# openai/Video-Pre-Training

Hardware: AMD Instinct MI355X
Metric: frames/sec (fwd) [+ bc_step.ms_per_step], 2x policy, 128x128x3 seq=128 (higher is better)
Workload: dtype bf16; 1 GPU; foundation-model-2x policy forward (IMPALA CNN + 4-layer banded transformer + heads), batch=64 seq=128 uint8 128x128x3 frames per GPU, KV memory carried, random-init weights; global_batch=64, seq_len=128, parallelism=dp1 replicas (no collective in forward; BC step: gradient all-reduce)

## Files before the change

video-pre-training_amd/csrc/vpt_conv3x3_fwd.hip:

```cpp
#include "vpt_conv3x3_tile.h"
#include <type_traits>
#ifndef VPT_EPI_NO_CLAMP_RELU
#define VPT_EPI_NO_CLAMP_RELU 0
#endif
#if defined(VPT_CONV_PROFILE) && defined(VPT_CONV_FWD_ABLATE)
#define FWD_NO_DMA (VPT_CONV_FWD_ABLATE == 1 || VPT_CONV_FWD_ABLATE == 4)
#define FWD_NO_HALO (VPT_CONV_FWD_ABLATE == 2 || VPT_CONV_FWD_ABLATE == 4)
#else
#define FWD_NO_DMA 0
#define FWD_NO_HALO 0
#endif
template <int U> __device__ __forceinline__ f32x4 ac_get(const f32x16& v) {
  return __builtin_shufflevector(v, v, 4 * U, 4 * U + 1, 4 * U + 2, 4 * U + 3);
}
template <int U> __device__ __forceinline__ void ac_set(f32x16& v, const f32x4 c) {
  const f32x16 w = __builtin_shufflevector(c, c, 0, 1, 2, 3, -1, -1, -1, -1, -1, -1, -1, -1, -1, -1, -1, -1);
  if constexpr (U == 0) v = __builtin_shufflevector(v, w, 16, 17, 18, 19, 4, 5, 6, 7, 8, 9, 10, 11, 12, 13, 14, 15);
  else if constexpr (U == 1) v = __builtin_shufflevector(v, w, 0, 1, 2, 3, 16, 17, 18, 19, 8, 9, 10, 11, 12, 13, 14, 15);
  else if constexpr (U == 2) v = __builtin_shufflevector(v, w, 0, 1, 2, 3, 4, 5, 6, 7, 16, 17, 18, 19, 12, 13, 14, 15);
  else v = __builtin_shufflevector(v, w, 0, 1, 2, 3, 4, 5, 6, 7, 8, 9, 10, 11, 16, 17, 18, 19);
}

template <bool TRACE, int MODE, int TR = 16, bool HDMA = false>
__global__ __launch_bounds__(TR * 16, 2) void vpt_conv3x3_kernel(VptConv3x3Args a) {
// ... 29 lines not shown
  const int tilesX = a.W >> 4, tilesY = a.H / TR;
  const VptConvTile tile = conv_tile_decode(a.NT, tilesX, tilesY);
  const int nt = tile.nt, tx = tile.tx, ty = tile.ty, f = tile.f;
  const int tx0 = tx * 16, ty0 = ty * TR;
  const int NCB = a.Cin >> 5;
  const int HW = a.H * a.W;

  int a_loff[NA];
  unsigned a_gbyte[NA];
  unsigned a_inside = 0;
#pragma unroll
  for (int m = 0; m < NA; ++m) {
    const int q = tid + NTHR * m;
    const int P = ((q >> 5) << 3) + 2 * (q & 3) + ((q >> 4) & 1);
    const int part = 2 * ((q >> 3) & 1) + ((q >> 2) & 1);
    a_loff[m] = -1;
    a_gbyte[m] = 0u;
    if (P < HPIX) {
      const int hy = P / 18, hx = P - hy * 18;
      const int y = ty0 - 1 + hy, x = tx0 - 1 + hx;
      a_loff[m] = P * A_RS + part * 16 + 16 * (P & 1);
      if (y >= 0 && y < a.H && x >= 0 && x < a.W) {
        a_gbyte[m] = (unsigned)((y * a.W + x) * 32 + part * 8) * 2u;
        a_inside |= 1u << m;
      }
    }
  }
  const op16_t* xplane = a.x + (size_t)f * NCB * HW * 32;
  constexpr int H16_STR = (NTHR / 4) * A_RS;
  static_assert(((NA - 2) * NTHR + NTHR - 1) / 32 * 8 + 7 < HPIX, "all chunks but a thread's last are inside the halo");
  const int a_l0 = a_loff[0];
  const bool a_lastok = a_loff[NA - 1] >= 0;
  const op16_t* wbase = a.wpk + (size_t)nt * NCB * 9 * 4096 + (size_t)(w * 64 + lane) * 8;
  unsigned char* bdst = smem + A_SZ + w * 1024;
  unsigned hv[6] = {0u, 0u, 0u, 0u, 0u, 0u};
  if constexpr (HDMA) {
#pragma unroll
    for (int n = 0; n < 6; ++n) {
      const int s = (n < 5 ? (4 * n + w) * 64 : (H_BUF - 1024) / 16) + lane;
      const int P = s >> 2, hy = P / 18, hx = P - 18 * hy;
      const int q = (s & 3) ^ ((hx >> 2) & 3);
      const int y = ty0 - 1 + hy, x = tx0 - 1 + hx;
      hv[n] = (y >= 0 && y < a.H && x >= 0 && x < a.W) ? (unsigned)((y * a.W + x) * 64 + q * 16) : H_OOB;
    }
  }
  const unsigned h_wbytes = (unsigned)NCB * 9u * (unsigned)H_SLOT, h_xbytes = (unsigned)NCB * (unsigned)HW * 64u;
  const op16_t* const h_wptr = a.wpk + (size_t)nt * NCB * 9 * 4096;
  const __amdgpu_buffer_rsrc_t hwrs = __builtin_amdgcn_make_buffer_rsrc((void*)h_wptr, 0, HDMA ? h_wbytes : 0u, 0x00020000);
  const __amdgpu_buffer_rsrc_t hxrs = __builtin_amdgcn_make_buffer_rsrc((void*)xplane, 0, HDMA ? h_xbytes : 0u, 0x00020000);
  const int h_wvoff = (w * 64 + lane) * 16;
  unsigned char* const rdst = smem + w * 1024;
  int h_wso = 0, h_rpi = 0;

#define GLDS16(m_)                                                                                        \
  do { if (POOL) { if (!FWD_NO_DMA) GLDS(m_); } else if ((m_) < NDMA && !FWD_NO_DMA)                      \
  __builtin_amdgcn_raw_ptr_buffer_load_lds(wrs, (__attribute__((address_space(3))) void*)(bd_ + (m_) * (NWAVE * 1024)), 16, wvoff, \
                                           (s_ + 1) * B_BYTES + (m_) * (NWAVE * 1024), 0, 0); } while (0)
#define XA16(m_) do { if (!FWD_NO_HALO) XA(m_); } while (0)
#define HALO_WR16(m_) do { if ((m_) < NA - 1 || a_lastok) *(u32x4*)(smem + a_l0 + (m_) * H16_STR) = ((a_inside >> (m_)) & 1u) ? areg[m_] : zero4; } while (0)
#define PA(j_, dy_, dx_) fp[j_] = *(const __attribute__((address_space(3))) op16x8*)((((dx_) & 1) ? aLo : aLe) + (((j_) + (dy_)) * 18 + (dx_)) * A_RS)
#define WB(tap_, u_, boff_) fw[(u_) & 1] = *(const __attribute__((address_space(3))) op16x8*)((((u_) & 1) ? bW1 : bW0) + (boff_) + (tap_) * (128 * 64) + ((u_) >> 1) * (32 * 64))
#define M16A(j_, u_) ac_set<(u_)>(ac[j_], VPT_MFMA_16X16X32(fw[(u_) & 1], fp[j_], ac_get<(u_)>(ac[j_]), 0, 0, 0))
#define G16(MM_, u_, WLD, X)                                                                              \
  do {                                                                                                    \
    MM_(0, u_); WLD; SB();                                                                                \
    MM_(1, u_); SB();                                                                                     \
    MM_(2, u_); SB();                                                                                     \
    MM_(3, u_); X; SB();                                                                                  \
    MM_(4, u_); SB();                                                                                     \
    MM_(5, u_); SB();                                                                                     \
    MM_(6, u_); SB();                                                                                     \
    MM_(7, u_); SB();                                                                                     \
  } while (0)
#define G16R(MM_, WLD, X, ndy_, ndx_)                                                                     \
  do {                                                                                                    \
    MM_(0, 3); SB(); WLD; PA(0, ndy_, ndx_); SB();                                                              \
    MM_(1, 3); SB(); PA(1, ndy_, ndx_); SB();                                                                   \
    MM_(2, 3); SB(); PA(2, ndy_, ndx_); SB();                                                                   \
    MM_(3, 3); SB(); PA(3, ndy_, ndx_); X; SB();                                                                \
    MM_(4, 3); SB(); PA(4, ndy_, ndx_); SB();                                                                   \
    MM_(5, 3); SB(); PA(5, ndy_, ndx_); SB();                                                                   \
    MM_(6, 3); SB(); PA(6, ndy_, ndx_); SB();                                                                   \
    MM_(7, 3); SB(); PA(7, ndy_, ndx_); SB();                                                                   \
  } while (0)
#define TAP16(MM_, dy_, dx_, X0, X1, X2, X3)                                                              \
  do {                                                                                                    \
    G16(MM_, 0, WB(dx_, 1, boff_), X0);                                                                   \
    G16(MM_, 1, WB(dx_, 2, boff_), X1);                                                                   \
    G16(MM_, 2, WB(dx_, 3, boff_), X2);                                                                   \
    G16R(MM_, WB((dx_) + 1, 0, boff_), X3, dy_, (dx_) + 1);                                               \
  } while (0)
#define EPI_LD16(ptr_, j_, n2_) (*(const u32x4*)((const char*)((ptr_) + cbase[n2_]) + (voff16 + (unsigned)(j_) * gj_b)))
#define XR16(j_) do { rq16[j_][0] = EPI_LD16(resp, j_, 0); rq16[j_][1] = EPI_LD16(resp, j_, 1); } while (0)
#define XR16L(j_) do { rq16[j_][0] = *(const u32x4*)((const char*)(resp + cbase[0]) + (voff16_l + (unsigned)(j_) * gj_b)); rq16[j_][1] = *(const u32x4*)((const char*)(resp + cbase[1]) + (voff16_l + (unsigned)(j_) * gj_b)); } while (0)
#define CONV_STEP16(cb_, dy_, NEXT_DY, PRE_A, WR_A, PRE_R, LAST)                                          \
  do {                                                                                                    \
    const int s_ = (cb_) * 3 + (dy_);                                                                     \
    const int boff_ = (s_ & 1) * B_BYTES, noff_ = B_BYTES - boff_;                                        \
    const op16_t* wp_ = wbase + (size_t)(s_ + 1) * 12288;      \
    unsigned char* bd_ = bdst + noff_;                                                                    \
    const unsigned cbo_ = (unsigned)((cb_) + 1) * (unsigned)HW * 64u;                 \
    if (LAST) {                                                                                           \
      TAP16(M16A, dy_, 0, NOP_(), NOP_(), NOP_(), NOP_());                                                \
    } else {                                                                                              \
      TAP16(M16A, dy_, 0, GLDS16(0), GLDS16(1), GLDS16(2), GLDS16(3));                                          \
    }                                                                                                     \
    if (PRE_A) {                                                                                          \
      TAP16(M16A, dy_, 1, GLDS16(4), GLDS16(5), do { XA16(0); XA16(1); } while (0), XA16(2));             \
      G16(M16A, 0, WB(2, 1, boff_), do { XA16(3); XA16(4); } while (0));                                  \
      G16(M16A, 1, WB(2, 2, boff_), XA16(5));                                                             \
      G16(M16A, 2, WB(2, 3, boff_), NOP_());                                                              \
      if (NA == 6) WAIT_BARRIER(6); else WAIT_BARRIER(5);                                                 \
    } else if ((PRE_R) && HAS_RES) {                                                                      \
      TAP16(M16A, dy_, 1, GLDS16(4), GLDS16(5), XR16(0), NOP_());                                           \
      G16(M16A, 0, WB(2, 1, boff_), NOP_());                                                              \
      G16(M16A, 1, WB(2, 2, boff_), NOP_());                                                              \
      G16(M16A, 2, WB(2, 3, boff_), NOP_());                                                              \
      WAIT_BARRIER(2);                                                                                         \
    } else {                                                                                              \
      if (LAST) TAP16(M16A, dy_, 1, NOP_(), NOP_(), NOP_(), NOP_());                                      \
      else TAP16(M16A, dy_, 1, GLDS16(4), GLDS16(5), NOP_(), NOP_());                                       \
      G16(M16A, 0, WB(2, 1, boff_), NOP_());                                                              \
      G16(M16A, 1, WB(2, 2, boff_), NOP_());                                                              \
      G16(M16A, 2, WB(2, 3, boff_), NOP_());                                                              \
      WAIT_BARRIER(0);                                                                                    \
    }                                                                                                     \
    if (WR_A) {    \
      _Pragma("unroll") for (int m_ = 0; m_ < 4; ++m_) {                                                  \
        if (!FWD_NO_HALO) HALO_WR16(m_); SB();                                                            \
        if (m_ + 4 < NA && !FWD_NO_HALO) HALO_WR16(m_ + 4);                                                         \
        SB(); if (m_ == 0) M16A(0, 3); else if (m_ == 1) M16A(1, 3); else if (m_ == 2) M16A(2, 3); else M16A(3, 3); SB();                                                                        \
      }                                                                                                   \
      WAIT_BARRIER(0);                                                                                    \
      WB(0, 0, noff_); PA(0, 0, 0); PA(1, 0, 0); PA(2, 0, 0); PA(3, 0, 0); SB();                          \
      M16A(4, 3); SB(); PA(4, 0, 0); SB();                                                                      \
      M16A(5, 3); SB(); PA(5, 0, 0); SB();                                                                      \
      M16A(6, 3); SB(); PA(6, 0, 0); SB();                                                                      \
      M16A(7, 3); SB(); PA(7, 0, 0); SB();                                                                      \
    } else if (LAST) {                                                                                    \
      M16A(0, 3); M16A(1, 3); M16A(2, 3); M16A(3, 3); M16A(4, 3); M16A(5, 3); M16A(6, 3); M16A(7, 3);                                    \
    } else {                                                                                              \
      G16R(M16A, WB(0, 0, noff_), NOP_(), NEXT_DY, 0);                                                    \
    }                                                                                                     \
  } while (0)
#define HWP(lp_, m_, rs_)                                                                                 \
  do { if (!FWD_NO_DMA) __builtin_amdgcn_raw_ptr_buffer_load_lds(rs_, (__attribute__((address_space(3))) void*)(rdst + ((((lp_) & 3) * H_SLOT) ^ h_rpi) + (m_) * 4096), \
                                           16, h_wvoff, h_wso + (lp_) * H_SLOT + (m_) * 4096, 0, 0); } while (0)
#define HXP_(n_, img_, rs_, cbo_)                                                                         \
  __builtin_amdgcn_raw_ptr_buffer_load_lds(rs_, (__attribute__((address_space(3))) void*)(smem + H_RING + (img_) * H_BUF + ((n_) < 5 ? w * 1024 + (n_) * 4096 : H_BUF - 1024)), \
                                           16, hv[n_], cbo_, 0, 0)
#define HXP(n_, img_, rs_, cbo_) do { if (!FWD_NO_HALO) HXP_(n_, img_, rs_, cbo_); } while (0)
#define HPA(j_, l_) fp[j_] = *(const __attribute__((address_space(3))) op16x8*)(((l_) % 3 == 0 ? aH0 : ((l_) % 3 == 1 ? aH1 : aH2)) + (((l_) % 18) >= 9 ? H_BUF : 0) + ((j_) + ((l_) % 9) / 3) * (18 * 64))
#define HWB(l_, u_) fw[(u_) & 1] = *(const __attribute__((address_space(3))) op16x8*)((((l_) & 2) ? (((u_) & 1) ? bWh1 : bWh0) : (((u_) & 1) ? bWl1 : bWl0)) + ((l_) & 1) * H_SLOT + ((u_) >> 1) * (32 * 64))
#define HG(l_, u_, X) G16(M16A, u_, HWB(l_, (u_) + 1), X)
#define HGR(l_, X)                                                                                        \
  do {                                                                                                    \
    M16A(0, 3); SB(); HWB((l_) + 1, 0); HPA(0, (l_) + 1); SB();                                           \
    M16A(1, 3); SB(); HPA(1, (l_) + 1); SB();                                                             \
    M16A(2, 3); SB(); HPA(2, (l_) + 1); SB();                                                             \
    M16A(3, 3); SB(); HPA(3, (l_) + 1); X; SB();                                                          \
    M16A(4, 3); SB(); HPA(4, (l_) + 1); SB();                                                             \
    M16A(5, 3); SB(); HPA(5, (l_) + 1); SB();                                                             \
    M16A(6, 3); SB(); HPA(6, (l_) + 1); SB();                                                             \
    M16A(7, 3); SB(); HPA(7, (l_) + 1); SB();                                                             \
  } while (0)
#define HSTEP(k_, X1, X2, X3, X4, X5, X6, X7, WAITB, X0N)                                                 \
  do {                                                                                                    \
    HG(2 * (k_), 0, X1); HG(2 * (k_), 1, X2); HG(2 * (k_), 2, X3); HGR(2 * (k_), X4);                     \
    HG(2 * (k_) + 1, 0, X5); HG(2 * (k_) + 1, 1, X6); HG(2 * (k_) + 1, 2, X7);                            \
    WAITB;                                                                                                \
    HGR(2 * (k_) + 1, X0N);                                                                               \
  } while (0)
#define EO16(j_) ((j_) == 0 ? eo_top : ((j_) == 7 ? eo_bot : 3 * 128))
#define LOAD_KK16(c_)                                                                                     \
  do {                                                                                                    \
    const float* kp_ = kk16 + EO16((c_) >> 1) + ((c_) & 1) * 32;                                          \
    kq[(c_) & 1][0] = *(const f32x4*)kp_; kq[(c_) & 1][1] = *(const f32x4*)(kp_ + 4);                     \
  } while (0)

  u32x4 areg[NA];
  const u32x4 zero4 = {0u, 0u, 0u, 0u};

  if constexpr (HDMA) {
    if (!FWD_NO_DMA) { HWP(0, 0, hwrs); HWP(0, 1, hwrs); HWP(1, 0, hwrs); HWP(1, 1, hwrs); }
    else { for (int t_ = 0; t_ < 4; ++t_) { __builtin_amdgcn_raw_ptr_buffer_load_lds(hwrs, (__attribute__((address_space(3))) void*)(rdst + t_ * H_SLOT), 16, h_wvoff, t_ * H_SLOT, 0, 0);
                                            __builtin_amdgcn_raw_ptr_buffer_load_lds(hwrs, (__attribute__((address_space(3))) void*)(rdst + t_ * H_SLOT + 4096), 16, h_wvoff, t_ * H_SLOT + 4096, 0, 0); } }
    HXP_(0, 0, hxrs, 0); HXP_(1, 0, hxrs, 0); HXP_(2, 0, hxrs, 0); HXP_(3, 0, hxrs, 0); HXP_(4, 0, hxrs, 0); HXP_(5, 0, hxrs, 0);
    if (FWD_NO_HALO) {
      const unsigned cb1_ = (unsigned)HW * 64u;
      HXP_(0, 1, hxrs, cb1_); HXP_(1, 1, hxrs, cb1_); HXP_(2, 1, hxrs, cb1_); HXP_(3, 1, hxrs, cb1_); HXP_(4, 1, hxrs, cb1_); HXP_(5, 1, hxrs, cb1_);
    }
  } else {
  ISSUE_B(0, 0);
#pragma unroll
  for (int m = 0; m < NA; ++m) areg[m] = *(const u32x4*)((const char*)xplane + a_gbyte[m]);
  }
  float mean = 0.f, rstd = 1.f;
  const float* esa = a.edge_sa;
  if (a.kk_frame) {
    rstd = a.rs_frame[f];
    esa = a.kk_frame + (size_t)f * 9 * a.CoutPad;
  } else {
    frame_mean_rstd(a.stats_in, f, a.inv_count_in, mean, rstd);
  }
  rstd = __builtin_bit_cast(float, __builtin_amdgcn_readfirstlane(__builtin_bit_cast(int, rstd)));
  mean = __builtin_bit_cast(float, __builtin_amdgcn_readfirstlane(__builtin_bit_cast(int, mean)));
  {
    float* kk = (float*)(smem + KK_O);
    constexpr int NKK = (9 * 128 + NTHR - 1) / NTHR;
    float ksa[NKK], ksg[NKK];
#pragma unroll
    for (int k = 0; k < NKK; ++k) {
      const int idx = tid + NTHR * k;
      const int o = (idx >> 7) * a.CoutPad + nt * 128 + (idx & 127);
      ksa[k] = (idx < 9 * 128) ? esa[o] : 0.f;
      ksg[k] = (idx < 9 * 128) ? a.edge_sg[o] : 0.f;
    }
#pragma unroll
    for (int k = 0; k < NKK; ++k) {
      const int idx = tid + NTHR * k;
      if (idx < 9 * 128) kk[idx] = (ksa[k] - rstd * mean * ksg[k]) * RELU_S;
    }
  }
  float res_s = 1.f;
  if (RES_AFF) {
    res_s = a.res_scale[f];
    if (tid < 128) ((float*)(smem + BT_O))[tid] = (nt * 128 + tid < a.Cout) ? a.res_bias[(size_t)f * a.Cout + nt * 128 + tid] : 0.f;
  }
  if constexpr (HDMA) {
    asm volatile("s_waitcnt vmcnt(0)" ::: "memory");
  } else {
#pragma unroll
    for (int m = 0; m < NA; ++m) HALO_WR16(m);
  }
  __syncthreads();

  f32x16 ac[8];
  f32x16 zero16;
#pragma unroll
  for (int r = 0; r < 16; ++r) zero16[r] = 0.f;

  const int hi = lane >> 5, l31 = lane & 31;
  const unsigned char* aL = smem + ((wm * 8 + sub_row(l31)) * 18 + (l31 & 15)) * A_RS + hi * 16;
  const int bsw = (l31 >> 2) & 3;
  const unsigned char* bL0 = smem + A_SZ + (wn * 64 + l31) * 64 + (((0 + hi) ^ bsw) << 4);
  const unsigned char* bL1 = smem + A_SZ + (wn * 64 + l31) * 64 + (((2 + hi) ^ bsw) << 4);
  (void)aL; (void)bL0; (void)bL1;

  const int c16 = lane & 15, q16 = lane >> 4;
  const int pcol = (c16 < 4) ? 2 * c16 : ((c16 < 12) ? 2 * (c16 - 4) + 1 : 2 * (c16 - 8));
  typedef const __attribute__((address_space(3))) unsigned char* lds_cptr;
  lds_cptr aLe = (lds_cptr)smem + ((wm * 8) * 18 + pcol) * A_RS + q16 * 16 + 16 * (pcol & 1);
  lds_cptr aLo = (lds_cptr)smem + ((wm * 8) * 18 + pcol) * A_RS + q16 * 16 + 16 * (1 - (pcol & 1));
  lds_cptr bW0 = (lds_cptr)smem + A_SZ + (wn * 64 + 8 * (c16 >> 2) + (c16 & 3)) * 64 + ((q16 ^ ((2 * (c16 >> 2)) & 3)) << 4);
  lds_cptr bW1 = (lds_cptr)smem + A_SZ + (wn * 64 + 8 * (c16 >> 2) + 4 + (c16 & 3)) * 64 + ((q16 ^ ((2 * (c16 >> 2) + 1) & 3)) << 4);
  if constexpr (!HDMA) { asm volatile("" : "+v"(aLe), "+v"(aLo), "+v"(bW0), "+v"(bW1)); }
#define HA_BASE(dx_) ((lds_cptr)smem + H_RING + ((wm * 8) * 18 + pcol + (dx_)) * 64 + ((q16 ^ (((pcol + (dx_)) >> 2) & 3)) << 4))
  lds_cptr aH0 = HA_BASE(0), aH1 = HA_BASE(1), aH2 = HA_BASE(2);
#undef HA_BASE
  lds_cptr bWl0 = (lds_cptr)smem + (wn * 64 + 8 * (c16 >> 2) + (c16 & 3)) * 64 + ((q16 ^ ((2 * (c16 >> 2)) & 3)) << 4);
  lds_cptr bWl1 = (lds_cptr)smem + (wn * 64 + 8 * (c16 >> 2) + 4 + (c16 & 3)) * 64 + ((q16 ^ ((2 * (c16 >> 2) + 1) & 3)) << 4);
  lds_cptr bWh0 = bWl0 + 2 * H_SLOT, bWh1 = bWl1 + 2 * H_SLOT;
  int h_swap = 2 * H_SLOT;
  if constexpr (HDMA) { asm volatile("" : "+v"(aH0), "+v"(aH1), "+v"(aH2), "+v"(bWl0), "+v"(bWl1), "+v"(bWh0), "+v"(bWh1)); }

  const int CB_out = a.Cout >> 5;
  const int cb0 = nt * 4 + wn * 2;
  const bool nvalid[2] = {(cb0 + 0) < CB_out, (cb0 + 1) < CB_out};
  size_t cbase[2];
#pragma unroll
  for (int n2 = 0; n2 < 2; ++n2) cbase[n2] = (size_t)(f * CB_out + (nvalid[n2] ? cb0 + n2 : 0)) * HW * 32;
  const unsigned voff16 = (unsigned)(((ty0 + wm * 8) * a.W + tx0 + pcol) * 32 + 8 * q16) * 2u;
  const unsigned gj_b = (unsigned)a.W * 64u;
  u32x4 rq16[8][2];

  const op16_t* resp = a.res;
  op16x8 fp[8], fw[2];
  const __amdgpu_buffer_rsrc_t wrs = __builtin_amdgcn_make_buffer_rsrc((void*)(a.wpk + (size_t)nt * NCB * 9 * 4096), 0, NCB * 9 * 8192, 0x00020000);
  const int wvoff = (w * 64 + lane) * 16;

  if (TRACE) t_trace[1] = wall_clock64();
  if constexpr (HDMA) {
    if (CONV_ABLATE != 2) {
      HWP(2, 0, hwrs);
      HWB(0, 0);
#pragma unroll
      for (int j = 0; j < 8; ++j) HPA(j, 0);
      SB();
#pragma unroll
      for (int j = 0; j < 8; ++j) ac[j] = zero16;
      const int NPASS = NCB >> 1;
#pragma unroll 1
      for (int ps = 0; ps < NPASS; ++ps) {
        const bool more = ps + 1 < NPASS;
        const __amdgpu_buffer_rsrc_t hwrs_n = __builtin_amdgcn_make_buffer_rsrc((void*)h_wptr, 0, more ? h_wbytes : 0u, 0x00020000);
        const __amdgpu_buffer_rsrc_t hxrs_n = __builtin_amdgcn_make_buffer_rsrc((void*)xplane, 0, more ? h_xbytes : 0u, 0x00020000);
        const unsigned cbB = (unsigned)(2 * ps + 1) * (unsigned)HW * 64u, cbA = cbB + (unsigned)HW * 64u;
        HSTEP(0, HWP(2, 1, hwrs), HWP(3, 0, hwrs), HWP(3, 1, hwrs), NOP_(), NOP_(), NOP_(), NOP_(), WAIT_BARRIER(0), HWP(4, 0, hwrs));
        HSTEP(1, HWP(4, 1, hwrs), HWP(5, 0, hwrs), HWP(5, 1, hwrs), HXP(0, 1, hxrs, cbB), HXP(1, 1, hxrs, cbB), HXP(2, 1, hxrs, cbB), HXP(3, 1, hxrs, cbB), WAIT_BARRIER(4), HWP(6, 0, hwrs));
        HSTEP(2, HWP(6, 1, hwrs), HWP(7, 0, hwrs), HWP(7, 1, hwrs), HXP(4, 1, hxrs, cbB), HXP(5, 1, hxrs, cbB), NOP_(), NOP_(), WAIT_BARRIER(2), HWP(8, 0, hwrs));
        HSTEP(3, HWP(8, 1, hwrs), HWP(9, 0, hwrs), HWP(9, 1, hwrs), NOP_(), NOP_(), NOP_(), NOP_(), WAIT_BARRIER(0), HWP(10, 0, hwrs));
        HSTEP(4, HWP(10, 1, hwrs), HWP(11, 0, hwrs), HWP(11, 1, hwrs), NOP_(), NOP_(), NOP_(), NOP_(), WAIT_BARRIER(0), HWP(12, 0, hwrs));
        HSTEP(5, HWP(12, 1, hwrs), HWP(13, 0, hwrs), HWP(13, 1, hwrs), HXP(0, 0, hxrs_n, cbA), HXP(1, 0, hxrs_n, cbA), HXP(2, 0, hxrs_n, cbA), HXP(3, 0, hxrs_n, cbA), WAIT_BARRIER(4), HWP(14, 0, hwrs));
        HSTEP(6, HWP(14, 1, hwrs), HWP(15, 0, hwrs), HWP(15, 1, hwrs), HXP(4, 0, hxrs_n, cbA), HXP(5, 0, hxrs_n, cbA), NOP_(), NOP_(), WAIT_BARRIER(2), HWP(16, 0, hwrs));
        if constexpr (HAS_RES) {
          HSTEP(7, HWP(16, 1, hwrs), HWP(17, 0, hwrs), HWP(17, 1, hwrs), XR16(0), NOP_(), NOP_(), NOP_(), WAIT_BARRIER(2), HWP(18, 0, hwrs_n));
        } else {
          HSTEP(7, HWP(16, 1, hwrs), HWP(17, 0, hwrs), HWP(17, 1, hwrs), NOP_(), NOP_(), NOP_(), NOP_(), WAIT_BARRIER(0), HWP(18, 0, hwrs_n));
        }
        HSTEP(8, HWP(18, 1, hwrs_n), HWP(19, 0, hwrs_n), HWP(19, 1, hwrs_n), NOP_(), NOP_(), NOP_(), NOP_(), WAIT_BARRIER(0), HWP(20, 0, hwrs_n));
        h_wso += 18 * H_SLOT;
        h_rpi ^= 2 * H_SLOT;
        bWl0 += h_swap; bWl1 += h_swap; bWh0 -= h_swap; bWh1 -= h_swap;
        h_swap = -h_swap;
      }
      asm volatile("s_waitcnt vmcnt(0)" ::: "memory");
    } else {
#pragma unroll
      for (int j = 0; j < 8; ++j) ac[j] = zero16;
      __syncthreads();
    }
  } else {
    if (CONV_ABLATE != 2) {
      WB(0, 0, 0);
#pragma unroll
      for (int j = 0; j < 8; ++j) PA(j, 0, 0);
      SB();
#pragma unroll
      for (int j = 0; j < 8; ++j) ac[j] = zero16;
#pragma unroll 1
      for (int cb = 0; cb + 1 < NCB; ++cb) {
        CONV_STEP16(cb, 0, 1, true, false, false, false);
        CONV_STEP16(cb, 1, 2, false, false, false, false);
        CONV_STEP16(cb, 2, 0, false, true, false, false);
      }
      CONV_STEP16(NCB - 1, 0, 1, false, false, !TRACE, false);
      CONV_STEP16(NCB - 1, 1, 2, false, false, false, false);
      CONV_STEP16(NCB - 1, 2, 0, false, false, false, true);
    } else {
#pragma unroll
      for (int j = 0; j < 8; ++j) ac[j] = zero16;
      __syncthreads();
    }
  }

  if (TRACE) t_trace[2] = wall_clock64();
  if (CONV_ABLATE == 1) {
    float t = 0.f;
#pragma unroll
    for (int j = 0; j < 8; ++j)
#pragma unroll
      for (int r = 0; r < 16; ++r) t += ac[j][r];
    if (t == 12345.678f) a.y[0] = (vpt_op16)t;
    return;
  }
  if (HAS_RES && (TRACE || CONV_ABLATE == 2)) XR16(0);
  SB();

  f32x2 s_sum2 = {0.f, 0.f}, s_sq2 = {0.f, 0.f};
  int lane_l = lane;
  asm volatile("" : "+v"(lane_l));
  const int c16_l = lane_l & 15, q16_l = lane_l >> 4;
  const int pcol_l = (c16_l < 4) ? 2 * c16_l : ((c16_l < 12) ? 2 * (c16_l - 4) + 1 : 2 * (c16_l - 8));
  const unsigned voff16_l = (unsigned)(((ty0 + wm * 8) * a.W + tx0 + pcol_l) * 32 + 8 * q16_l) * 2u;
  const int x16_ = tx0 + pcol_l;
  const int ex16 = (x16_ == 0) ? 0 : ((x16_ == a.W - 1) ? 2 : 1);
  const int eo_top = (ty0 + wm * 8 == 0) ? 0 : 3 * 128, eo_bot = (ty0 + wm * 8 + 7 == a.H - 1) ? 6 * 128 : 3 * 128;
  const float* kk16 = (const float*)(smem + KK_O) + ex16 * 128 + wn * 64 + 8 * q16_l;
  auto epilogue16 = [&](auto nv_) __attribute__((always_inline)) {
    constexpr int NV = decltype(nv_)::value;
    u32x4 outv[8][2];
    f32x4 kq[2][2];
    LOAD_KK16(0);
    SB();
    const f32x2 zero2 = {0.f, 0.f};
    const f32x2 rstd2 = {rstd * RELU_S, rstd * RELU_S}, ress2 = {res_s, res_s};
    const f32x2 relu_inv2 = {RELU_INV, RELU_INV};
    const float* btab = (const float*)(smem + BT_O) + wn * 64 + 8 * q16_l;
#pragma unroll
    for (int j = 0; j < 8; ++j) {
      if (HAS_RES && j == 0) XR16L(1);
      if (HAS_RES && j < 6) XR16L(j + 2);
      SB();
#pragma unroll
      for (int n2 = 0; n2 < 2; ++n2) {
        if (2 * j + n2 < 15) { LOAD_KK16(2 * j + n2 + 1); SB(); }
        if (n2 >= NV) continue;
        f32x4 bq[2];
        if (RES_AFF) {
          bq[0] = *(const f32x4*)(btab + n2 * 32); bq[1] = *(const f32x4*)(btab + n2 * 32 + 4);
          SB();
        }
        u32x2 pk[2];
#pragma unroll
        for (int h = 0; h < 2; ++h) {
          f32x2 v01 = {ac[j][8 * n2 + 4 * h + 0], ac[j][8 * n2 + 4 * h + 1]}, v23 = {ac[j][8 * n2 + 4 * h + 2], ac[j][8 * n2 + 4 * h + 3]};
          const f32x4 k4 = kq[n2][h];
          const f32x2 k01 = {k4.x, k4.y}, k23 = {k4.z, k4.w};
          if (PACKED_RELU) {
            v01 = rstd2 * v01 + k01;
            v23 = rstd2 * v23 + k23;
          } else if (CLAMP_RELU) {
            v01 = pk_fma_clamp01(rstd2, v01, k01);
            v23 = pk_fma_clamp01(rstd2, v23, k23);
          } else {
            v01 = __builtin_elementwise_max(rstd2 * v01 + k01, zero2);
            v23 = __builtin_elementwise_max(rstd2 * v23 + k23, zero2);
          }
          if (HAS_RES) {
            const uint32_t ra = h ? rq16[j][n2].z : rq16[j][n2].x, rb = h ? rq16[j][n2].w : rq16[j][n2].y;
            const f32x2 r01 = {op16_lo_to_f32(ra), op16_hi_to_f32(ra)}, r23 = {op16_lo_to_f32(rb), op16_hi_to_f32(rb)};
            if (RES_AFF) {
              const f32x4 b4 = bq[h];
              const f32x2 b01 = {b4.x, b4.y}, b23 = {b4.z, b4.w};
              if (CLAMP_RELU) {
                v01 = ress2 * r01 + __builtin_elementwise_fma(v01, relu_inv2, b01);
                v23 = ress2 * r23 + __builtin_elementwise_fma(v23, relu_inv2, b23);
              } else {
                v01 = ress2 * r01 + (v01 + b01);
                v23 = ress2 * r23 + (v23 + b23);
              }
            } else if (CLAMP_RELU) {
              v01 = __builtin_elementwise_fma(v01, relu_inv2, r01);
              v23 = __builtin_elementwise_fma(v23, relu_inv2, r23);
            } else {
              v01 += r01;
              v23 += r23;
            }
          }
          pk[h].x = pack_op16x2(v01.x, v01.y);
          pk[h].y = pack_op16x2(v23.x, v23.y);
          if (PACKED_RELU) {
            pk[h].x = relu_op16x2(pk[h].x);
            pk[h].y = relu_op16x2(pk[h].y);
          }
          s_sum2.x = dot2_op16(pk[h].x, OP16_ONE2, s_sum2.x);
          s_sum2.y = dot2_op16(pk[h].y, OP16_ONE2, s_sum2.y);
          s_sq2.x = dot2_op16(pk[h].x, pk[h].x, s_sq2.x);
          s_sq2.y = dot2_op16(pk[h].y, pk[h].y, s_sq2.y);
        }
        outv[j][n2] = u32x4{pk[0].x, pk[0].y, pk[1].x, pk[1].y};
      }
    }
#pragma unroll
    for (int j = 0; j < 8; ++j)
#pragma unroll
      for (int n2 = 0; n2 < NV; ++n2)
        *(u32x4*)((char*)(a.y + cbase[n2]) + (voff16_l + (unsigned)j * gj_b)) = outv[j][n2];
  };
  if constexpr (POOL) {
    const __attribute__((address_space(4))) VptConv3x3Args* late = (const __attribute__((address_space(4))) VptConv3x3Args*)__builtin_amdgcn_kernarg_segment_ptr();
    asm volatile("" : "+s"(late));
    int tid_p = threadIdx.x;
    asm volatile("" : "+v"(tid_p));
    const int tid = tid_p, lane = tid_p & 63;
    vpt_op16* const seam_r_p = late->seam_r;
    vpt_op16* const seam_c_p = late->seam_c;
    vpt_op16* const pool_mask_p = late->pool_mask;
    double* const chs_out_p = late->chs_out;
    __syncthreads();
    {
      const f32x2 zero2 = {0.f, 0.f};
      const f32x2 rstd2 = {rstd, rstd};
#pragma unroll
      for (int j = 0; j < 8; ++j) {
        const float* ke = kk16 + EO16(j);
        unsigned char* dst = smem + ((wm * 8 + j) * 16 + pcol_l) * PT_RS + (wn * 64 + 8 * q16_l) * 2;
#pragma unroll
        for (int n2 = 0; n2 < 2; ++n2) {
          if (!nvalid[n2]) continue;
          u32x2 pk[2];
#pragma unroll
          for (int h = 0; h < 2; ++h) {
            const f32x4 k4 = *(const f32x4*)(ke + n2 * 32 + 4 * h);
            const f32x2 k01 = {k4.x, k4.y}, k23 = {k4.z, k4.w};
            f32x2 v01 = {ac[j][8 * n2 + 4 * h + 0], ac[j][8 * n2 + 4 * h + 1]}, v23 = {ac[j][8 * n2 + 4 * h + 2], ac[j][8 * n2 + 4 * h + 3]};
            if (PMASK) {
              v01 = __builtin_elementwise_max(rstd2 * v01 + k01, zero2);
              v23 = __builtin_elementwise_max(rstd2 * v23 + k23, zero2);
            } else {
              v01 = rstd2 * v01 + k01;
              v23 = rstd2 * v23 + k23;
            }
            pk[h].x = pack_op16x2(v01.x, v01.y);
            pk[h].y = pack_op16x2(v23.x, v23.y);
          }
          *(u32x4*)(dst + n2 * 64) = u32x4{pk[0].x, pk[0].y, pk[1].x, pk[1].y};
        }
      }
    }
    __syncthreads();
    typedef short i16x8 __attribute__((ext_vector_type(8)));
    const int PH = a.H >> 1, PW = a.W >> 1;
    const bool top_open = ty0 > 0, left_open = tx0 > 0;
    float p_sum = 0.f, p_sq = 0.f;
    float c1[8], c2[8];
#pragma unroll
    for (int k = 0; k < 8; ++k) { c1[k] = 0.f; c2[k] = 0.f; }
#pragma unroll
    for (int it = 0; it < 4; ++it) {
      const int item = tid + 256 * it;
      const int oct = item & 15, pi = (item >> 4) & 7, pj = item >> 7;
      const int cg = nt * 128 + oct * 8;
      const unsigned char* src = smem + oct * 16;
      i16x8 mx = {0, 0, 0, 0, 0, 0, 0, 0};
      i16x8 vv[PMASK ? 9 : 1];
#pragma unroll
      for (int dy = -1; dy <= 1; ++dy) {
        const int r = 2 * pj + dy;
#pragma unroll
        for (int dx = -1; dx <= 1; ++dx) {
          const int c = 2 * pi + dx;
          const i16x8 v = *(const i16x8*)(src + (max(r, 0) * 16 + max(c, 0)) * PT_RS);
          mx = __builtin_elementwise_max(mx, v);
          if (PMASK) vv[PMASK ? (dy + 1) * 3 + dx + 1 : 0] = v;
        }
      }
      if constexpr (PMASK) {
        const u32x4 mxu = __builtin_bit_cast(u32x4, mx);
        u32x4 mk = {0u, 0u, 0u, 0u};
        const uint32_t one2 = 0x00010001u, two2 = 0x00020002u;
#pragma unroll
        for (int k = 0; k < 9; ++k) {
          const u32x4 vk = __builtin_bit_cast(u32x4, vv[k]);
          const bool inside = (2 * pj + k / 3 - 1 >= 0) && (2 * pi + k % 3 - 1 >= 0);
#pragma unroll
          for (int j = 0; j < 4; ++j) {
            uint32_t t = inside ? (vk[j] ^ mxu[j]) : 0xffffffffu, b, m2;
            asm("v_pk_min_u16 %0, %1, %2" : "=v"(b) : "v"(t), "s"(one2));
            asm("v_pk_mad_u16 %0, %1, %2, %3" : "=v"(m2) : "v"(mk[j]), "s"(two2), "v"(b));
            mk[j] = m2;
          }
        }
        if (cg < a.Cout) {
          const size_t moff = ((size_t)(f * CB_out + (cg >> 5)) * PH * PW + (size_t)(((ty0 >> 1) + pj) * PW + (tx0 >> 1) + pi)) * 32 + (cg & 31);
          *(u32x4*)(pool_mask_p + moff) = mk;
        }
      }
      if (cg < a.Cout) {
        u32x4 mv = __builtin_bit_cast(u32x4, mx);
        const size_t off = ((size_t)(f * CB_out + (cg >> 5)) * PH * PW + (size_t)(((ty0 >> 1) + pj) * PW + (tx0 >> 1) + pi)) * 32 + (cg & 31);
        const bool complete = (pj > 0 || !top_open) && (pi > 0 || !left_open);
        if (complete) {
#pragma unroll
          for (int k = 0; k < 4; ++k) {
            p_sum = dot2_op16(mv[k], OP16_ONE2, p_sum);
            p_sq = dot2_op16(mv[k], mv[k], p_sq);
          }
          if (a.out_gain) {
            float vals[8];
            unpack8(mv, vals);
            const f32x4 g0 = *(const f32x4*)(a.out_gain + cg), g1 = *(const f32x4*)(a.out_gain + cg + 4);
            vals[0] *= g0.x; vals[1] *= g0.y; vals[2] *= g0.z; vals[3] *= g0.w; vals[4] *= g1.x; vals[5] *= g1.y; vals[6] *= g1.z; vals[7] *= g1.w;
            mv = pack8(vals);
          }
          if (chs_out_p) {
            float q[8];
            unpack8(mv, q);
#pragma unroll
            for (int k = 0; k < 8; ++k) { c1[k] += q[k]; c2[k] = fmaf(q[k], q[k], c2[k]); }
          }
        }
        *(u32x4*)(a.y + off) = mv;
      }
    }
    {
      const int oct = tid & 15, q = tid >> 4;
      const int cg = nt * 128 + oct * 8;
      if (cg < a.Cout) {
        if (ty0 + 16 < a.H) {
          const u32x4 v = *(const u32x4*)(smem + (15 * 16 + q) * PT_RS + oct * 16);
          *(u32x4*)(seam_r_p + ((size_t)((f * CB_out + (cg >> 5)) * tilesY + ty) * a.W + tx0 + q) * 32 + (cg & 31)) = v;
        }
        if (tx0 + 16 < a.W) {
          const u32x4 v = *(const u32x4*)(smem + (q * 16 + 15) * PT_RS + oct * 16);
          *(u32x4*)(seam_c_p + ((size_t)((f * CB_out + (cg >> 5)) * tilesX + tx) * a.H + ty0 + q) * 32 + (cg & 31)) = v;
        }
      }
    }
    s_sum2.x = p_sum; s_sum2.y = 0.f; s_sq2.x = p_sq; s_sq2.y = 0.f;
    if (chs_out_p) {
      float* scr = (float*)(smem + KK_O);
#pragma unroll
      for (int k = 0; k < 8; ++k) {
        c1[k] += __shfl_xor(c1[k], 16, 64); c1[k] += __shfl_xor(c1[k], 32, 64);
        c2[k] += __shfl_xor(c2[k], 16, 64); c2[k] += __shfl_xor(c2[k], 32, 64);
      }
      if (lane < 16) {
#pragma unroll
        for (int k = 0; k < 8; ++k) { scr[(w * 16 + lane) * 16 + k] = c1[k]; scr[(w * 16 + lane) * 16 + 8 + k] = c2[k]; }
      }
      __syncthreads();
      {
        const int o = tid >> 4, k = tid & 15;
        const float t = (scr[(0 * 16 + o) * 16 + k] + scr[(1 * 16 + o) * 16 + k]) + (scr[(2 * 16 + o) * 16 + k] + scr[(3 * 16 + o) * 16 + k]);
        const int ch = nt * 128 + o * 8 + (k & 7);
        if (ch < a.Cout) atomicAdd(chs_out_p + ((size_t)f * a.Cout + ch) * 2 + (k >> 3), (double)t);
      }
    }
  } else {
    if (nvalid[1]) epilogue16(std::integral_constant<int, 2>{});
    else if (nvalid[0]) epilogue16(std::integral_constant<int, 1>{});
  }
#undef GLDS16
#undef XA16
#undef HALO_WR16
#undef PA
#undef WB
#undef M16A
#undef G16
#undef G16R
#undef TAP16
#undef EPI_LD16
#undef XR16
#undef XR16L
#undef CONV_STEP16
#undef HWP
#undef HXP_
#undef HXP
#undef HPA
#undef HWB
#undef HG
#undef HGR
#undef HSTEP
#undef EO16
#undef LOAD_KK16
  float s_sum = s_sum2.x + s_sum2.y, s_sq = s_sq2.x + s_sq2.y;
  if (a.stats_out) {
    float* red = (float*)(smem + KK_O + KK_BYTES);
    s_sum = wave_sum(s_sum);
    s_sq = wave_sum(s_sq);
    if (lane == 0) { red[w] = s_sum; red[NWAVE + w] = s_sq; }
    __syncthreads();
    if (tid == 0) {
      float t1 = (red[0] + red[1]) + (red[2] + red[3]), t2 = (red[NWAVE] + red[NWAVE + 1]) + (red[NWAVE + 2] + red[NWAVE + 3]);
      if (NWAVE == 8) {
        t1 += (red[4] + red[5]) + (red[6] + red[7]);
        t2 += (red[12] + red[13]) + (red[14] + red[15]);
      }
      atomicAdd(a.stats_out + 2 * f, (double)t1);
      atomicAdd(a.stats_out + 2 * f + 1, (double)t2);
    }
  }
  if (TRACE && tid == 0) {
    long long* t = a.trace + (size_t)blockIdx.x * 12;
    t[0] = t_trace[0]; t[1] = t_trace[1]; t[2] = t_trace[2]; t[3] = wall_clock64(); t[4] = cu_key; t[5] = 0;
    for (int k = 0; k < 5; ++k) t[6 + k] = 0;
  }
}

void vpt_conv3x3_fwd_launch(const VptConv3x3Args* a, int mode, int variant, long grid, int extra_lds, hipStream_t stream) {
#ifdef VPT_CONV_PROFILE
  static bool lds_attr_set = false;
  if (extra_lds > 0 && !lds_attr_set) {
    (void)hipFuncSetAttribute((const void*)vpt_conv3x3_kernel<false, 0>, hipFuncAttributeMaxDynamicSharedMemorySize, extra_lds);
    (void)hipFuncSetAttribute((const void*)vpt_conv3x3_kernel<false, 1>, hipFuncAttributeMaxDynamicSharedMemorySize, extra_lds);
    lds_attr_set = true;
  }
#endif
#define LAUNCH_(T_, M_) hipLaunchKernelGGL((vpt_conv3x3_kernel<T_, M_>), dim3((unsigned)grid), dim3(256), extra_lds, stream, *a)
#define LAUNCH32_(M_) hipLaunchKernelGGL((vpt_conv3x3_kernel<false, M_, 32>), dim3((unsigned)grid), dim3(512), 0, stream, *a)
#define LAUNCHH_(M_) hipLaunchKernelGGL((vpt_conv3x3_kernel<false, M_, 16, true>), dim3((unsigned)grid), dim3(256), 0, stream, *a)
  if (variant == 1) { if (mode == 0) LAUNCH32_(0); else if (mode == 1) LAUNCH32_(1); else LAUNCH32_(5); }
  else if (variant == 2) { if (mode == 0) LAUNCHH_(0); else if (mode == 1) LAUNCHH_(1); else if (mode == 4) LAUNCHH_(4); else LAUNCHH_(5); }
  else if (a->trace) { if (mode == 0) LAUNCH_(true, 0); else LAUNCH_(true, 1); }
  else if (mode == 0) LAUNCH_(false, 0); else if (mode == 1) LAUNCH_(false, 1); else if (mode == 4) LAUNCH_(false, 4); else if (mode == 5) LAUNCH_(false, 5); else LAUNCH_(false, 7);
#undef LAUNCH_
#undef LAUNCH32_
#undef LAUNCHH_
}

template <bool MASK>
__global__ __launch_bounds__(256) void vpt_pool_seam_kernel(VptPoolSeamArgs a) {
  typedef short i16x8 __attribute__((ext_vector_type(8)));
  __shared__ float red[4][4][18];
  const int tid = threadIdx.x, lane = tid & 63, w = tid >> 6;
  const int PH = a.H >> 1, PW = a.W >> 1, TY = a.H >> 4, TX = a.W >> 4;
  const int n_row = (TY - 1) * PW;
  const int col_len = PH - (TY - 1);
  const int n_pix = n_row + (TX - 1) * col_len;
  const int cb = blockIdx.x % a.CB, f = blockIdx.x / a.CB;
  const int oct = tid & 3;
  const size_t plane = (size_t)(f * a.CB + cb);
  float s_sum = 0.f, s_sq = 0.f;
  float c1[8], c2[8];
  float gv[8];
#pragma unroll
  for (int k = 0; k < 8; ++k) { c1[k] = 0.f; c2[k] = 0.f; gv[k] = a.gain ? a.gain[cb * 32 + oct * 8 + k] : 1.f; }
  for (int pix = tid >> 2; pix < n_pix; pix += 64) {
    int J, I;
    if (pix < n_row) { J = (pix / PW + 1) * 8; I = pix % PW; }
    else {
      const int q = pix - n_row, t = q / col_len, k = q - t * col_len;
      I = (t + 1) * 8;
      J = (k == 0) ? 0 : (k - 1) / 7 * 8 + (k - 1) % 7 + 1;
    }
    vpt_op16* yp = a.y + (plane * PH * PW + (size_t)(J * PW + I)) * 32 + oct * 8;
    i16x8 m = *(const i16x8*)yp;
    const i16x8 m_in = m;
    i16x8 sv[6];
    bool have[6] = {false, false, false, false, false, false};
    if ((J & 7) == 0 && J > 0) {
      const vpt_op16* sr = a.seam_r + ((plane * TY + (J >> 3) - 1) * a.W) * 32 + oct * 8;
#pragma unroll
      for (int dx = -1; dx <= 1; ++dx) {
        const int x = 2 * I + dx;
        if (x >= 0) {
          const i16x8 v = *(const i16x8*)(sr + (size_t)x * 32);
          m = __builtin_elementwise_max(m, v);
          if (MASK) { sv[dx + 1] = v; have[dx + 1] = true; }
        }
      }
    }
    if ((I & 7) == 0 && I > 0) {
      const vpt_op16* sc = a.seam_c + ((plane * TX + (I >> 3) - 1) * a.H) * 32 + oct * 8;
#pragma unroll
      for (int dy = -1; dy <= 1; ++dy) {
        const int y = 2 * J + dy;
        if (y >= 0) {
          const i16x8 v = *(const i16x8*)(sc + (size_t)y * 32);
          m = __builtin_elementwise_max(m, v);
          if (MASK) { sv[3 + dy + 1] = v; have[3 + dy + 1] = true; }
        }
      }
    }
    if constexpr (MASK) {
      typedef unsigned short u16x8 __attribute__((ext_vector_type(8)));
      unsigned short* mp = (unsigned short*)a.mask + (plane * PH * PW + (size_t)(J * PW + I)) * 32 + oct * 8;
      u16x8 mk = *(const u16x8*)mp;
#pragma unroll
      for (int c = 0; c < 8; ++c) {
        unsigned bits = (m_in[c] == m[c]) ? (unsigned)mk[c] : 0x1ffu;
#pragma unroll
        for (int q = 0; q < 6; ++q) {
          const int k = q < 3 ? q : 3 * (q - 3);
          if (have[q] && sv[q][c] == m[c]) bits &= ~(1u << (8 - k));
        }
        mk[c] = (unsigned short)bits;
      }
      *(u16x8*)mp = mk;
    }
    float vals[8];
    u32x4 mv = __builtin_bit_cast(u32x4, m);
    unpack8(mv, vals);
#pragma unroll
    for (int k = 0; k < 8; ++k) { s_sum += vals[k]; s_sq = fmaf(vals[k], vals[k], s_sq); }
    if (a.gain) {
#pragma unroll
      for (int k = 0; k < 8; ++k) vals[k] *= gv[k];
      mv = pack8(vals);
      unpack8(mv, vals);
    }
    *(u32x4*)yp = mv;
#pragma unroll
    for (int k = 0; k < 8; ++k) { c1[k] += vals[k]; c2[k] = fmaf(vals[k], vals[k], c2[k]); }
  }
#pragma unroll
  for (int off = 4; off < 64; off <<= 1) {
#pragma unroll
    for (int k = 0; k < 8; ++k) { c1[k] += __shfl_xor(c1[k], off, 64); c2[k] += __shfl_xor(c2[k], off, 64); }
    s_sum += __shfl_xor(s_sum, off, 64); s_sq += __shfl_xor(s_sq, off, 64);
  }
  if (lane < 4) {
#pragma unroll
    for (int k = 0; k < 8; ++k) { red[w][lane][k] = c1[k]; red[w][lane][8 + k] = c2[k]; }
    red[w][lane][16] = s_sum; red[w][lane][17] = s_sq;
  }
  __syncthreads();
  if (tid < 64 && a.chs_out) {
    const int o = tid >> 4, k = tid & 15;
    const float t = (red[0][o][k] + red[1][o][k]) + (red[2][o][k] + red[3][o][k]);
    atomicAdd(a.chs_out + ((size_t)f * a.CB * 32 + cb * 32 + o * 8 + (k & 7)) * 2 + (k >> 3), (double)t);
  }
  if (tid >= 64 && tid < 66 && a.stats_out) {
    const int k = 16 + (tid - 64);
    float t = 0.f;
#pragma unroll
// ... 17 lines not shown
```

Measured before the change: 80600 frames/s.

## Peel first and last halo-DMA passes to drop accumulator zeroing and overlap residual loads

Restructures the halo-DMA conv main loop into a peeled first pass, a steady-state loop and a peeled last pass. The first pass uses MFMA with a zero accumulator instead of zeroing the accumulators up front. The last pass skips prefetching the next pass's weights and halo. It also issues the residual loads (XR16 0-2) inside the tail MMA groups instead of in the epilogue. This is meant to cut zero-init instructions and useless tail prefetches, and to hide residual load latency behind compute. The cost is a larger unrolled code body and more instruction-cache and register pressure.

```diff
diff --git a/video-pre-training_amd/csrc/vpt_conv3x3_fwd.hip b/video-pre-training_amd/csrc/vpt_conv3x3_fwd.hip
--- a/video-pre-training_amd/csrc/vpt_conv3x3_fwd.hip
+++ b/video-pre-training_amd/csrc/vpt_conv3x3_fwd.hip
@@ -205,24 +205,74 @@
 #define HXP(n_, img_, rs_, cbo_) do { if (!FWD_NO_HALO) HXP_(n_, img_, rs_, cbo_); } while (0)
 #define HPA(j_, l_) fp[j_] = *(const __attribute__((address_space(3))) op16x8*)(((l_) % 3 == 0 ? aH0 : ((l_) % 3 == 1 ? aH1 : aH2)) + (((l_) % 18) >= 9 ? H_BUF : 0) + ((j_) + ((l_) % 9) / 3) * (18 * 64))
 #define HWB(l_, u_) fw[(u_) & 1] = *(const __attribute__((address_space(3))) op16x8*)((((l_) & 2) ? (((u_) & 1) ? bWh1 : bWh0) : (((u_) & 1) ? bWl1 : bWl0)) + ((l_) & 1) * H_SLOT + ((u_) >> 1) * (32 * 64))
-#define HG(l_, u_, X) G16(M16A, u_, HWB(l_, (u_) + 1), X)
-#define HGR(l_, X)                                                                                        \
-  do {                                                                                                    \
-    M16A(0, 3); SB(); HWB((l_) + 1, 0); HPA(0, (l_) + 1); SB();                                           \
-    M16A(1, 3); SB(); HPA(1, (l_) + 1); SB();                                                             \
-    M16A(2, 3); SB(); HPA(2, (l_) + 1); SB();                                                             \
-    M16A(3, 3); SB(); HPA(3, (l_) + 1); X; SB();                                                          \
-    M16A(4, 3); SB(); HPA(4, (l_) + 1); SB();                                                             \
-    M16A(5, 3); SB(); HPA(5, (l_) + 1); SB();                                                             \
-    M16A(6, 3); SB(); HPA(6, (l_) + 1); SB();                                                             \
-    M16A(7, 3); SB(); HPA(7, (l_) + 1); SB();                                                             \
-  } while (0)
-#define HSTEP(k_, X1, X2, X3, X4, X5, X6, X7, WAITB, X0N)                                                 \
-  do {                                                                                                    \
-    HG(2 * (k_), 0, X1); HG(2 * (k_), 1, X2); HG(2 * (k_), 2, X3); HGR(2 * (k_), X4);                     \
-    HG(2 * (k_) + 1, 0, X5); HG(2 * (k_) + 1, 1, X6); HG(2 * (k_) + 1, 2, X7);                            \
+#define M16Z(j_, u_) do { ac_set<(u_)>(ac[j_], VPT_MFMA_16X16X32(fw[(u_) & 1], fp[j_], zero4f, 0, 0, 0)); if ((u_) == 0) asm volatile("" : "+v"(ac[j_])); } while (0)
+#define HG(MM_, l_, u_, X) G16(MM_, u_, HWB(l_, (u_) + 1), X)
+#define HGR(MM_, l_, X)                                                                                   \
+  do {                                                                                                    \
+    MM_(0, 3); SB(); HWB((l_) + 1, 0); HPA(0, (l_) + 1); SB();                                            \
+    MM_(1, 3); SB(); HPA(1, (l_) + 1); SB();                                                              \
+    MM_(2, 3); SB(); HPA(2, (l_) + 1); SB();                                                              \
+    MM_(3, 3); SB(); HPA(3, (l_) + 1); X; SB();                                                           \
+    MM_(4, 3); SB(); HPA(4, (l_) + 1); SB();                                                              \
+    MM_(5, 3); SB(); HPA(5, (l_) + 1); SB();                                                              \
+    MM_(6, 3); SB(); HPA(6, (l_) + 1); SB();                                                              \
+    MM_(7, 3); SB(); HPA(7, (l_) + 1); SB();                                                              \
+  } while (0)
+#define HGL()                                                                                             \
+  do {                                                                                                    \
+    M16A(0, 3); SB(); M16A(1, 3); SB(); M16A(2, 3); SB(); M16A(3, 3); SB();                               \
+    M16A(4, 3); SB(); M16A(5, 3); SB(); M16A(6, 3); SB(); M16A(7, 3); SB();                               \
+  } while (0)
+#define HSTEP(MM0_, k_, X1, X2, X3, X4, X5, X6, X7, WAITB, LASTG)                                         \
+  do {                                                                                                    \
+    HG(MM0_, 2 * (k_), 0, X1); HG(MM0_, 2 * (k_), 1, X2); HG(MM0_, 2 * (k_), 2, X3); HGR(MM0_, 2 * (k_), X4); \
+    HG(M16A, 2 * (k_) + 1, 0, X5); HG(M16A, 2 * (k_) + 1, 1, X6); HG(M16A, 2 * (k_) + 1, 2, X7);          \
     WAITB;                                                                                                \
-    HGR(2 * (k_) + 1, X0N);                                                                               \
+    LASTG;                                                                                                \
+  } while (0)
+#define HPASS(MM0_, K_, ps_)                                                                              \
+  do {                                                                                                    \
+    const unsigned cbB = (unsigned)(2 * (ps_) + 1) * (unsigned)HW * 64u, cbA = cbB + (unsigned)HW * 64u;    \
+    HSTEP(MM0_, 0, HWP(2, 1, hwrs), HWP(3, 0, hwrs), HWP(3, 1, hwrs), NOP_(), NOP_(), NOP_(), NOP_(), WAIT_BARRIER(0), HGR(M16A, 1, HWP(4, 0, hwrs))); \
+    HSTEP(M16A, 1, HWP(4, 1, hwrs), HWP(5, 0, hwrs), HWP(5, 1, hwrs), HXP(0, 1, hxrs, cbB), HXP(1, 1, hxrs, cbB), HXP(2, 1, hxrs, cbB), HXP(3, 1, hxrs, cbB), WAIT_BARRIER(4), HGR(M16A, 3, HWP(6, 0, hwrs))); \
+    HSTEP(M16A, 2, HWP(6, 1, hwrs), HWP(7, 0, hwrs), HWP(7, 1, hwrs), HXP(4, 1, hxrs, cbB), HXP(5, 1, hxrs, cbB), NOP_(), NOP_(), WAIT_BARRIER(2), HGR(M16A, 5, HWP(8, 0, hwrs))); \
+    HSTEP(M16A, 3, HWP(8, 1, hwrs), HWP(9, 0, hwrs), HWP(9, 1, hwrs), NOP_(), NOP_(), NOP_(), NOP_(), WAIT_BARRIER(0), HGR(M16A, 7, HWP(10, 0, hwrs))); \
+    HSTEP(M16A, 4, HWP(10, 1, hwrs), HWP(11, 0, hwrs), HWP(11, 1, hwrs), NOP_(), NOP_(), NOP_(), NOP_(), WAIT_BARRIER(0), HGR(M16A, 9, HWP(12, 0, hwrs))); \
+    if constexpr ((K_) != 2) {                                                                            \
+      HSTEP(M16A, 5, HWP(12, 1, hwrs), HWP(13, 0, hwrs), HWP(13, 1, hwrs), HXP(0, 0, hxrs_n, cbA), HXP(1, 0, hxrs_n, cbA), HXP(2, 0, hxrs_n, cbA), HXP(3, 0, hxrs_n, cbA), WAIT_BARRIER(4), HGR(M16A, 11, HWP(14, 0, hwrs))); \
+      HSTEP(M16A, 6, HWP(14, 1, hwrs), HWP(15, 0, hwrs), HWP(15, 1, hwrs), HXP(4, 0, hxrs_n, cbA), HXP(5, 0, hxrs_n, cbA), NOP_(), NOP_(), WAIT_BARRIER(2), HGR(M16A, 13, HWP(16, 0, hwrs))); \
+      HSTEP(M16A, 7, HWP(16, 1, hwrs), HWP(17, 0, hwrs), HWP(17, 1, hwrs), NOP_(), NOP_(), NOP_(), NOP_(), WAIT_BARRIER(0), HGR(M16A, 15, HWP(18, 0, hwrs_n))); \
+      HSTEP(M16A, 8, HWP(18, 1, hwrs_n), HWP(19, 0, hwrs_n), HWP(19, 1, hwrs_n), NOP_(), NOP_(), NOP_(), NOP_(), WAIT_BARRIER(0), HGR(M16A, 17, HWP(20, 0, hwrs_n))); \
+    } else {                                                                                              \
+      HSTEP(M16A, 5, HWP(12, 1, hwrs), HWP(13, 0, hwrs), HWP(13, 1, hwrs), NOP_(), NOP_(), NOP_(), NOP_(), WAIT_BARRIER(0), HGR(M16A, 11, HWP(14, 0, hwrs))); \
+      HSTEP(M16A, 6, HWP(14, 1, hwrs), HWP(15, 0, hwrs), HWP(15, 1, hwrs), NOP_(), NOP_(), NOP_(), NOP_(), WAIT_BARRIER(0), HGR(M16A, 13, HWP(16, 0, hwrs))); \
+      if constexpr (HAS_RES) {    \
+        HSTEP(M16A, 7, HWP(16, 1, hwrs), HWP(17, 0, hwrs), HWP(17, 1, hwrs), XR16(0), NOP_(), NOP_(), NOP_(), WAIT_BARRIER(2), HGR(M16A, 15, NOP_())); \
+      } else {                                                                                            \
+        HSTEP(M16A, 7, HWP(16, 1, hwrs), HWP(17, 0, hwrs), HWP(17, 1, hwrs), NOP_(), NOP_(), NOP_(), NOP_(), WAIT_BARRIER(0), HGR(M16A, 15, NOP_())); \
+      }                                                                                                   \
+      if constexpr (HAS_RES) {    \
+        HSTEP(M16A, 8, XR16(1), NOP_(), NOP_(), XR16(2), NOP_(), NOP_(), NOP_(), SB(), HGL());            \
+      } else {                                                                                            \
+        HSTEP(M16A, 8, NOP_(), NOP_(), NOP_(), NOP_(), NOP_(), NOP_(), NOP_(), SB(), HGL());              \
+      }                                                                                                   \
+    }                                                                                                     \
+  } while (0)
+#define HPASS_HEAD()                                                                                      \
+  do {                                                                                                    \
+     \
+    _Pragma("unroll") for (int j_ = 0; j_ < 8; ++j_) asm volatile("" : "=v"(ac[j_]));                     \
+    HWP(2, 0, hwrs);                                                                                      \
+    HWB(0, 0);                                                                                            \
+    _Pragma("unroll") for (int j_ = 0; j_ < 8; ++j_) HPA(j_, 0);                                          \
+    SB();                                                                                                 \
+  } while (0)
+#define HPASS_NEXT()                                                                                      \
+  do {                                                                                                    \
+    h_wso += 18 * H_SLOT;                                                                                 \
+    h_rpi ^= 2 * H_SLOT;                                                                                  \
+    bWl0 += h_swap; bWl1 += h_swap; bWh0 -= h_swap; bWh1 -= h_swap;                                       \
+    h_swap = -h_swap;                                                                                     \
   } while (0)
 #define EO16(j_) ((j_) == 0 ? eo_top : ((j_) == 7 ? eo_bot : 3 * 128))
 #define LOAD_KK16(c_)                                                                                     \
@@ -292,6 +342,7 @@
   f32x16 zero16;
 #pragma unroll
   for (int r = 0; r < 16; ++r) zero16[r] = 0.f;
+  const f32x4 zero4f = {0.f, 0.f, 0.f, 0.f};
 
   const int hi = lane >> 5, l31 = lane & 31;
   const unsigned char* aL = smem + ((wm * 8 + sub_row(l31)) * 18 + (l31 & 15)) * A_RS + hi * 16;
@@ -335,39 +386,27 @@
   if (TRACE) t_trace[1] = wall_clock64();
   if constexpr (HDMA) {
     if (CONV_ABLATE != 2) {
-      HWP(2, 0, hwrs);
-      HWB(0, 0);
-#pragma unroll
-      for (int j = 0; j < 8; ++j) HPA(j, 0);
-      SB();
-#pragma unroll
-      for (int j = 0; j < 8; ++j) ac[j] = zero16;
       const int NPASS = NCB >> 1;
-#pragma unroll 1
-      for (int ps = 0; ps < NPASS; ++ps) {
-        const bool more = ps + 1 < NPASS;
+      {
+        const bool more = NPASS > 1;
         const __amdgpu_buffer_rsrc_t hwrs_n = __builtin_amdgcn_make_buffer_rsrc((void*)h_wptr, 0, more ? h_wbytes : 0u, 0x00020000);
         const __amdgpu_buffer_rsrc_t hxrs_n = __builtin_amdgcn_make_buffer_rsrc((void*)xplane, 0, more ? h_xbytes : 0u, 0x00020000);
-        const unsigned cbB = (unsigned)(2 * ps + 1) * (unsigned)HW * 64u, cbA = cbB + (unsigned)HW * 64u;
-        HSTEP(0, HWP(2, 1, hwrs), HWP(3, 0, hwrs), HWP(3, 1, hwrs), NOP_(), NOP_(), NOP_(), NOP_(), WAIT_BARRIER(0), HWP(4, 0, hwrs));
-        HSTEP(1, HWP(4, 1, hwrs), HWP(5, 0, hwrs), HWP(5, 1, hwrs), HXP(0, 1, hxrs, cbB), HXP(1, 1, hxrs, cbB), HXP(2, 1, hxrs, cbB), HXP(3, 1, hxrs, cbB), WAIT_BARRIER(4), HWP(6, 0, hwrs));
-        HSTEP(2, HWP(6, 1, hwrs), HWP(7, 0, hwrs), HWP(7, 1, hwrs), HXP(4, 1, hxrs, cbB), HXP(5, 1, hxrs, cbB), NOP_(), NOP_(), WAIT_BARRIER(2), HWP(8, 0, hwrs));
-        HSTEP(3, HWP(8, 1, hwrs), HWP(9, 0, hwrs), HWP(9, 1, hwrs), NOP_(), NOP_(), NOP_(), NOP_(), WAIT_BARRIER(0), HWP(10, 0, hwrs));
-        HSTEP(4, HWP(10, 1, hwrs), HWP(11, 0, hwrs), HWP(11, 1, hwrs), NOP_(), NOP_(), NOP_(), NOP_(), WAIT_BARRIER(0), HWP(12, 0, hwrs));
-        HSTEP(5, HWP(12, 1, hwrs), HWP(13, 0, hwrs), HWP(13, 1, hwrs), HXP(0, 0, hxrs_n, cbA), HXP(1, 0, hxrs_n, cbA), HXP(2, 0, hxrs_n, cbA), HXP(3, 0, hxrs_n, cbA), WAIT_BARRIER(4), HWP(14, 0, hwrs));
-        HSTEP(6, HWP(14, 1, hwrs), HWP(15, 0, hwrs), HWP(15, 1, hwrs), HXP(4, 0, hxrs_n, cbA), HXP(5, 0, hxrs_n, cbA), NOP_(), NOP_(), WAIT_BARRIER(2), HWP(16, 0, hwrs));
-        if constexpr (HAS_RES) {
-          HSTEP(7, HWP(16, 1, hwrs), HWP(17, 0, hwrs), HWP(17, 1, hwrs), XR16(0), NOP_(), NOP_(), NOP_(), WAIT_BARRIER(2), HWP(18, 0, hwrs_n));
-        } else {
-          HSTEP(7, HWP(16, 1, hwrs), HWP(17, 0, hwrs), HWP(17, 1, hwrs), NOP_(), NOP_(), NOP_(), NOP_(), WAIT_BARRIER(0), HWP(18, 0, hwrs_n));
-        }
-        HSTEP(8, HWP(18, 1, hwrs_n), HWP(19, 0, hwrs_n), HWP(19, 1, hwrs_n), NOP_(), NOP_(), NOP_(), NOP_(), WAIT_BARRIER(0), HWP(20, 0, hwrs_n));
-        h_wso += 18 * H_SLOT;
-        h_rpi ^= 2 * H_SLOT;
-        bWl0 += h_swap; bWl1 += h_swap; bWh0 -= h_swap; bWh1 -= h_swap;
-        h_swap = -h_swap;
-      }
-      asm volatile("s_waitcnt vmcnt(0)" ::: "memory");
+        HPASS_HEAD();
+        HPASS(M16Z, 0, 0);
+      }
+      if (NPASS > 1) {
+        const __amdgpu_buffer_rsrc_t hwrs_n = hwrs, hxrs_n = hxrs;
+        HPASS_NEXT();
+#pragma unroll 1
+        for (int ps = 1; ps + 1 < NPASS; ++ps) {
+          HPASS(M16A, 1, ps);
+          HPASS_NEXT();
+        }
+        HPASS(M16A, 2, NPASS - 1);
+      } else {
+        asm volatile("s_waitcnt vmcnt(0)" ::: "memory");
+        if constexpr (HAS_RES) { XR16(0); XR16(1); XR16(2); }
+      }
     } else {
 #pragma unroll
       for (int j = 0; j < 8; ++j) ac[j] = zero16;
@@ -407,7 +446,7 @@
     if (t == 12345.678f) a.y[0] = (vpt_op16)t;
     return;
   }
-  if (HAS_RES && (TRACE || CONV_ABLATE == 2)) XR16(0);
+  if (HAS_RES && (TRACE || CONV_ABLATE == 2)) { XR16(0); if (HDMA) { XR16(1); XR16(2); } }
   SB();
 
   f32x2 s_sum2 = {0.f, 0.f}, s_sq2 = {0.f, 0.f};
@@ -432,8 +471,8 @@
     const float* btab = (const float*)(smem + BT_O) + wn * 64 + 8 * q16_l;
 #pragma unroll
     for (int j = 0; j < 8; ++j) {
-      if (HAS_RES && j == 0) XR16L(1);
-      if (HAS_RES && j < 6) XR16L(j + 2);
+      if (HAS_RES && !HDMA && j == 0) XR16L(1);
+      if (HAS_RES && j < 6 && !(HDMA && j == 0)) XR16L(j + 2);
       SB();
 #pragma unroll
       for (int n2 = 0; n2 < 2; ++n2) {
@@ -676,6 +715,11 @@
 #undef HG
 #undef HGR
 #undef HSTEP
+#undef M16Z
+#undef HGL
+#undef HPASS
+#undef HPASS_NEXT
+#undef HPASS_HEAD
 #undef EO16
 #undef LOAD_KK16
   float s_sum = s_sum2.x + s_sum2.y, s_sq = s_sq2.x + s_sq2.y;
```

New measurement: 81010 frames/s (median of 6 runs). No clear change (+0.5%).
